# gunrock/graphblast

Hardware: NVIDIA H100
Metric: MTEPS (higher is better)
Workload: dtype f32

## Files before the change

### graphblast_b200/csrc/graphblas/backend/cuda/bfs_fused.hpp

```cpp
#ifndef GRAPHBLAS_BACKEND_CUDA_BFS_FUSED_HPP_
#define GRAPHBLAS_BACKEND_CUDA_BFS_FUSED_HPP_

#include "graphblas/backend/cuda/kernels/bfs_fused.cuh"

namespace graphblas {
namespace backend {

inline bool bfsFusedApplies(Descriptor* desc) {
  static const int enabled = getEnv("GB200_BFS_FUSED", 1);
  if (!enabled) return false;
  Desc_value mask_mode, outp, inp0, inp1;
  if (desc->get(GrB_MASK, &mask_mode) != GrB_SUCCESS) return false;
  desc->get(GrB_OUTP, &outp); desc->get(GrB_INP0, &inp0); desc->get(GrB_INP1, &inp1);
  return desc->struconly() && desc->opreuse() && desc->earlyexit() && desc->fusedmask() &&
         mask_mode == GrB_DEFAULT && outp == GrB_DEFAULT && inp0 == GrB_DEFAULT &&
         inp1 == GrB_DEFAULT && !desc->debug() && desc->timing_ != 1;
}

inline void bfsFusedStats(Descriptor* desc, Index n, unsigned long long out[6]) {
  for (int i = 0; i < 6; ++i) out[i] = 0ull;
  const size_t nwords = (static_cast<size_t>(n) + 31)/32;
  const size_t words_bytes = ((nwords*sizeof(unsigned int) + 255)/256)*256;
  if (desc->scratchSize(GB_SCRATCH_BFS) < 4*words_bytes + 256) return;
  unsigned char* base = reinterpret_cast<unsigned char*>(desc->scratch(GB_SCRATCH_BFS, 0));
  CUDA_CALL(cudaMemcpyAsync(out, base + 4*words_bytes + 6*sizeof(unsigned long long),
      6*sizeof(unsigned long long), cudaMemcpyDeviceToHost, gbStream()));
  runtime().sync();
}

template <typename a>
Info bfsFused(Vector<float>* v, const Matrix<a>* A, Index s, Descriptor* desc, int* depth) {
  SparseMatrix<a>* S = const_cast<SparseMatrix<a>*>(&A->sparse_);
  const Index n = S->nrows_;
  if (n != S->ncols_) return GrB_DIMENSION_MISMATCH;
  if (S->d_csrRowPtr_ == NULL || S->d_cscColPtr_ == NULL) return GrB_UNINITIALIZED_OBJECT;
  cudaStream_t stream = gbStream();
  CHECK(v->setStorage(GrB_DENSE));
  CHECK(v->dense_.allocateGpu());

  const int fw = 1;
  const Index* probe = pullMaxDegreeNeighbours(S, fw, S->d_cscColPtr_, S->d_cscRowInd_, n);

  const size_t nwords = (static_cast<size_t>(n) + 31)/32;
  const size_t words_bytes = ((nwords*sizeof(unsigned int) + 255)/256)*256;
  const size_t nchunks = (nwords + 31)/32;
  const size_t counters_bytes = GB_BFS_NCOUNTERS*sizeof(unsigned long long);
  const size_t heavy_bytes = GB_BFS_HEAVY_CAP*sizeof(Index);
  const size_t walk_bytes = nchunks*GB_BFS_CHUNK*sizeof(Index);
  const size_t lists_bytes = ((nchunks*(sizeof(int) + sizeof(Index)) + 255)/256)*256;
  const size_t level8_bytes = ((static_cast<size_t>(n) + 255)/256)*256;
  unsigned char* base = reinterpret_cast<unsigned char*>(desc->scratch(GB_SCRATCH_BFS,
      4*words_bytes + counters_bytes + heavy_bytes + walk_bytes + lists_bytes +
      level8_bytes));
  BfsFusedArgs args;
  args.push_ptr = S->d_csrRowPtr_;  args.push_ind = S->d_csrColInd_;
  args.pull_ptr = S->d_cscColPtr_;  args.pull_ind = S->d_cscRowInd_;
  args.pull_probe = probe;
  const bool same_structure = S->symmetric_ || S->d_cscColPtr_ == S->d_csrRowPtr_;
  args.pull_empty = pullEmptyRowBits(probe, n);
  args.push_empty = same_structure ? NULL : pullEmptyRowBits(
      pullFirstNeighbours(S, 0, S->d_csrRowPtr_, S->d_csrColInd_, n), n);
  args.n = n;
  args.source = s;
  args.max_levels = desc->max_niter_;
  args.switchpoint = desc->switchpoint();
  Desc_value mode;
  CHECK(desc->get(GrB_MXVMODE, &mode));
  args.mode = (mode == GrB_PUSHONLY) ? 1 : (mode == GrB_PULLONLY ? 2 : 0);
  args.levels = v->dense_.d_val_;
  args.visited[0] = reinterpret_cast<unsigned int*>(base);
  args.visited[1] = reinterpret_cast<unsigned int*>(base + words_bytes);
  args.frontier   = reinterpret_cast<unsigned int*>(base + 2*words_bytes);
  args.next       = reinterpret_cast<unsigned int*>(base + 3*words_bytes);
  args.counters   = reinterpret_cast<unsigned long long*>(base + 4*words_bytes);
  args.heavy      = reinterpret_cast<Index*>(base + 4*words_bytes + counters_bytes);
  args.walk       = reinterpret_cast<Index*>(base + 4*words_bytes + counters_bytes +
                                             heavy_bytes);
  args.walk_count = reinterpret_cast<int*>(base + 4*words_bytes + counters_bytes +
                                           heavy_bytes + walk_bytes);
  args.walk_chunks = reinterpret_cast<Index*>(args.walk_count + nchunks);
  args.level8     = base + 4*words_bytes + counters_bytes + heavy_bytes + walk_bytes +
                    lists_bytes;

  static const int trace = getEnv("GB200_BFS_TRACE", 0);
  args.trace = trace;
  args.prof_bytes = NULL;
  if (profiler().enabled) {
    profiler().ensureCells();
    args.prof_bytes = profiler().d_cells + GB_PROF_PULL_BOOL;
  }

  const bool push_only = (args.mode == 1);
  void (*kernel)(BfsFusedArgs) =
      push_only ? bfsFusedKernel<GB_BFS_PUSH_NT, GB_BFS_PUSH_MINB, false>
                : bfsFusedKernel<GB_BFS_NT, GB_BFS_MINB, true>;
  const int nt = push_only ? GB_BFS_PUSH_NT : GB_BFS_NT;
  static int resident_of[2] = {0, 0};
  int& resident = resident_of[push_only ? 1 : 0];
  if (resident == 0) {
    int per_sm = 0;
    CUDA_CALL(cudaOccupancyMaxActiveBlocksPerMultiprocessor(&per_sm, kernel, nt, 0));
    resident = per_sm*runtime().sm_count;
    if (resident < 1) return GrB_PANIC;
  }
  void* params[] = { &args };
  profiler().begin(GB_PROF_PULL_BOOL, stream);
  CUDA_CALL(cudaLaunchCooperativeKernel(reinterpret_cast<void*>(kernel),
      dim3(resident), dim3(nt), params, 0, stream));
  GB_KERNEL_CHECK();
  profiler().end(GB_PROF_PULL_BOOL, stream, 0.0);
  v->dense_.touched();
  if (trace) {
    unsigned long long cells[GB_BFS_NCOUNTERS];
    CUDA_CALL(cudaMemcpyAsync(cells, args.counters, sizeof(cells), cudaMemcpyDeviceToHost,
        stream));
    runtime().sync();
    const int levels = static_cast<int>(cells[6] < 15 ? cells[6] : 15);
    fprintf(stderr, "bfs trace: set-up %.1fus",
            1e-3*static_cast<double>((cells[12] >> 1) - cells[28]));
    for (int l = 1; l <= levels; ++l) {
      const unsigned long long start = cells[12 + l - 1] >> 1, end = cells[12 + l] >> 1;
      if (cells[12 + l] & 1ull)
        fprintf(stderr, " L%d pull %.1fus (scan %.1f walk %.1f, %llu walked, %llu listed)",
                l, 1e-3*static_cast<double>(end - start),
                1e-3*static_cast<double>(cells[44 + l] - start),
                1e-3*static_cast<double>(end - cells[44 + l]), cells[60 + l],
                cells[76 + l]);
      else
        fprintf(stderr, " L%d push %.1fus", l, 1e-3*static_cast<double>(end - start));
    }
    fprintf(stderr, " end-pass %.1fus\n", 1e-3*static_cast<double>(cells[29] - cells[30]));
  }
  if (depth != NULL) {
    const unsigned long long levels = runtime().fetch(args.counters + 6);
    *depth = static_cast<int>(levels);
    desc->lastmxv_ = GrB_PULLONLY;
  }
  return GrB_SUCCESS;
}

}
}

#endif
```

### graphblast_b200/csrc/graphblas/backend/cuda/kernels/bfs_fused.cuh

```cuda
#ifndef GRAPHBLAS_BACKEND_CUDA_KERNELS_BFS_FUSED_CUH_
#define GRAPHBLAS_BACKEND_CUDA_KERNELS_BFS_FUSED_CUH_

#include <cooperative_groups.h>

#include "graphblas/backend/cuda/kernels/common.cuh"

namespace graphblas {
namespace backend {

#ifndef GB_BFS_NT
#define GB_BFS_NT     512
#endif
#ifndef GB_BFS_MINB
#define GB_BFS_MINB   2
#endif
#ifndef GB_BFS_PUSH_NT
#define GB_BFS_PUSH_NT   768
#endif
#ifndef GB_BFS_PUSH_MINB
#define GB_BFS_PUSH_MINB 2
#endif
#ifndef GB_BFS_BATCH
#define GB_BFS_BATCH  4
#endif
#ifndef GB_BFS_WALK_STEP
#define GB_BFS_WALK_STEP 4
#endif
#ifndef GB_BFS_WALK_WARP
#define GB_BFS_WALK_WARP 32
#endif
#ifndef GB_BFS_WALK_INLINE
#define GB_BFS_WALK_INLINE 64
#endif
#define GB_BFS_HEAVY  2048
#define GB_BFS_HEAVY_CAP 4096
#define GB_BFS_CHUNK  1024

struct BfsFusedArgs {
  const Index* push_ptr;   const Index* push_ind;
  const Index* pull_ptr;   const Index* pull_ind;
  const Index* pull_probe;
  const unsigned int* pull_empty;
  const unsigned int* push_empty;
  int   trace;
  unsigned long long* prof_bytes;
  Index n;
  Index source;
  int   max_levels;
  float switchpoint;
  int   mode;
  float*        levels;
  unsigned char* level8;
  unsigned int* visited[2];
  unsigned int* frontier;
  unsigned int* next;
  unsigned long long* counters;
  Index*        heavy;
  Index*        walk;
  int*          walk_count;
  Index*        walk_chunks;
};
#define GB_BFS_NCOUNTERS 128

__device__ __forceinline__ unsigned long long bfsClockNs() {
  unsigned long long t;
  asm volatile("mov.u64 %0, %globaltimer;" : "=l"(t));
  return t;
}

__device__ __forceinline__ bool bfsClaim(unsigned int* visited, Index vtx) {
  const unsigned int bit = 1u << (vtx & 31);
  unsigned int* word = visited + (vtx >> 5);
  if (*reinterpret_cast<volatile unsigned int*>(word) & bit) return false;
  return (atomicOr(word, bit) & bit) == 0;
}

__device__ __forceinline__ void bfsSetLevel(const BfsFusedArgs& a, Index row, int lv) {
  if (lv < 255) {
    a.level8[row] = static_cast<unsigned char>(lv);
  } else {
    a.level8[row] = 255;
    a.levels[row] = static_cast<float>(lv);
  }
}

__device__ __forceinline__ Index bfsClaimChunk(unsigned long long* cell, int lane) {
  unsigned long long c = 0ull;
  if (lane == 0) c = atomicAdd(cell, 1ull);
  return static_cast<Index>(__shfl_sync(GB_FULL_MASK, c, 0));
}

__device__ __forceinline__ unsigned int* bfsVis(const BfsFusedArgs& a, int vsel) {
  return vsel ? a.visited[1] : a.visited[0];
}
__device__ __forceinline__ unsigned int* bfsVisOther(const BfsFusedArgs& a, int vsel) {
  return vsel ? a.visited[0] : a.visited[1];
}
__device__ __forceinline__ unsigned int* bfsF(const BfsFusedArgs& a, int fsel) {
  return fsel ? a.next : a.frontier;
}
__device__ __forceinline__ unsigned int* bfsN(const BfsFusedArgs& a, int fsel) {
  return fsel ? a.frontier : a.next;
}

__device__ __forceinline__ unsigned int bfsIsolated(const BfsFusedArgs& a, Index w) {
  return a.pull_empty[w] & (a.push_empty != NULL ? a.push_empty[w] : 0xffffffffu);
}

__device__ __forceinline__ bool bfsWalkRows(const BfsFusedArgs& a, int vsel, Index row,
                                            bool active, int lane, int& inspected) {
  Index k = 0, end = 0;
  if (active) {
    k = __ldg(a.pull_ptr + row);
    end = __ldg(a.pull_ptr + row + 1);
  }
  const Index stop = (end - k > GB_BFS_WALK_WARP + GB_BFS_WALK_STEP)
                     ? k + GB_BFS_WALK_STEP : end;
  bool found = false;
  while (k < stop && !found) {
    Index col[GB_BFS_WALK_STEP];
    unsigned int wv[GB_BFS_WALK_STEP];
#pragma unroll
    for (int u = 0; u < GB_BFS_WALK_STEP; ++u)
      col[u] = (k + u < stop) ? __ldg(a.pull_ind + k + u) : static_cast<Index>(-1);
#pragma unroll
    for (int u = 0; u < GB_BFS_WALK_STEP; ++u)
      wv[u] = (col[u] >= 0) ? bfsVis(a, vsel)[col[u] >> 5] : 0u;
#pragma unroll
    for (int u = 0; u < GB_BFS_WALK_STEP; ++u) {
      if (found || col[u] < 0) continue;
      ++inspected;
      found = (wv[u] >> (col[u] & 31)) & 1u;
    }
    k += GB_BFS_WALK_STEP;
  }
  unsigned int longs = __ballot_sync(GB_FULL_MASK, !found && k < end);
  while (longs != 0u) {
    const int src = __ffs(longs) - 1;
    longs &= longs - 1u;
    const Index lend = __shfl_sync(GB_FULL_MASK, end, src);
    bool hit = false;
    for (Index lk = __shfl_sync(GB_FULL_MASK, k, src); lk < lend && !hit; lk += 32) {
      bool v = false;
      if (lk + lane < lend) {
        const Index col = __ldg(a.pull_ind + lk + lane);
        v = (bfsVis(a, vsel)[col >> 5] >> (col & 31)) & 1u;
      }
      const unsigned int b = __ballot_sync(GB_FULL_MASK, v);
      hit = (b != 0u);
      if (lane == 0)
        inspected += hit ? __ffs(b) : (lend - lk < 32 ? lend - lk : 32);
    }
    if (lane == src) found = hit;
  }
  return found;
}

template <int NT, int MINB, bool PULL>
__global__ void __launch_bounds__(NT, MINB)
bfsFusedKernel(BfsFusedArgs a) {
  namespace cg = cooperative_groups;
  cg::grid_group grid = cg::this_grid();
  __shared__ int s_red[NT/32];
  __shared__ unsigned int s_found[PULL ? NT/32 : 1][PULL ? 32 : 1];

  const Index n = a.n;
  const Index nwords = (n + 31) >> 5;
  const int lane = threadIdx.x & 31;
  const Index gtid = blockIdx.x*NT + threadIdx.x;
  const Index gthreads = gridDim.x*NT;
  const Index gwarp = gtid >> 5;
  const Index gwarps = gthreads >> 5;
  const Index nchunks = (nwords + 31) >> 5;

  if (gtid == 0) a.counters[28] = bfsClockNs();
  if (gtid == 0) a.level8[a.source] = 1;
  for (Index w = gtid; w < nwords; w += gthreads) {
    const unsigned int seed = (w == (a.source >> 5)) ? (1u << (a.source & 31)) : 0u;
    a.visited[0][w] = seed | bfsIsolated(a, w);
    a.visited[1][w] = 0u; a.frontier[w] = seed; a.next[w] = 0u;
  }
  if (gtid < 12) a.counters[gtid] = 0ull;
  if (gtid >= 35 && gtid < 41) a.counters[gtid] = 0ull;
  if (gtid >= 60 && gtid < 76) a.counters[gtid] = 0ull;
  grid.sync();
  if (gtid == 0) a.counters[12] = bfsClockNs() << 1;

  int vsel = 0;
  int fsel = 0;
  unsigned int fcount = 1u;
  bool dense = PULL && (a.mode == 2);
  float prev_ratio = 0.f;
  int inspected = 0;
  int pushed_vertices = 0;
  unsigned int pushed_edges = 0u;
  int pull_levels = 0;
  int level = 1;

  for (; level <= a.max_levels && fcount > 0u; ++level) {
    if (PULL && a.mode == 0) {
      const float ratio = static_cast<float>(fcount)/static_cast<float>(n);
      if (!dense) {
        if (ratio > a.switchpoint && ratio > prev_ratio) dense = true; else prev_ratio = ratio;
      } else {
        if (ratio <= a.switchpoint && ratio < prev_ratio) dense = false; else prev_ratio = ratio;
      }
    }
    unsigned long long* const count_cell = a.counters + (level % 3);
    unsigned long long* const heavy_cell = a.counters + 3 + (level % 3);
    if (gtid == 0) {
      a.counters[(level + 1) % 3] = 0ull;
      a.counters[3 + (level + 1) % 3] = 0ull;
      a.counters[35 + (level + 1) % 3] = 0ull;
      a.counters[38 + (level + 1) % 3] = 0ull;
    }
    int found_here = 0;

    if (!dense) {
      for (Index w0 = gwarp*32; w0 < nwords; w0 += gwarps*32) {
        const Index mine = w0 + lane;
        unsigned int my_bits = (mine < nwords) ? bfsF(a, fsel)[mine] : 0u;
        if (my_bits != 0u) bfsF(a, fsel)[mine] = 0u;
        unsigned int pending = __ballot_sync(GB_FULL_MASK, my_bits != 0u);
        while (pending != 0u) {
          const int src_lane = __ffs(pending) - 1;
          pending &= pending - 1u;
          unsigned int bits = __shfl_sync(GB_FULL_MASK, my_bits, src_lane);
          const Index w = w0 + src_lane;
          while (bits != 0u) {
            const int b = __ffs(bits) - 1;
            bits &= bits - 1u;
            const Index u = w*32 + b;
            const Index beg = __ldg(a.push_ptr + u);
            const Index deg = __ldg(a.push_ptr + u + 1) - beg;
            if (lane == 0) { ++pushed_vertices; pushed_edges += deg; }
            if (deg > GB_BFS_HEAVY) {
              unsigned long long slot = 0ull;
              if (lane == 0) slot = atomicAdd(heavy_cell, 1ull);
              slot = __shfl_sync(GB_FULL_MASK, slot, 0);
              if (slot < GB_BFS_HEAVY_CAP) {
                if (lane == 0) a.heavy[slot] = u;
                continue;
              }
            }
            for (Index k = lane; k < deg; k += 32) {
              const Index nbr = __ldg(a.push_ind + beg + k);
              if (bfsClaim(bfsVis(a, vsel), nbr)) {
                bfsSetLevel(a, nbr, level + 1);
                atomicOr(bfsN(a, fsel) + (nbr >> 5), 1u << (nbr & 31));
                ++found_here;
              }
            }
          }
        }
      }
      grid.sync();
      const unsigned long long listed =
          *reinterpret_cast<volatile unsigned long long*>(heavy_cell);
      const int nheavy = (listed > GB_BFS_HEAVY_CAP) ? GB_BFS_HEAVY_CAP
                                                     : static_cast<int>(listed);
      if (nheavy > 0) {
        for (int h = 0; h < nheavy; ++h) {
          const Index u = a.heavy[h];
          const Index beg = __ldg(a.push_ptr + u);
          const Index deg = __ldg(a.push_ptr + u + 1) - beg;
          for (Index k = gtid; k < deg; k += gthreads) {
            const Index nbr = __ldg(a.push_ind + beg + k);
            if (bfsClaim(bfsVis(a, vsel), nbr)) {
              bfsSetLevel(a, nbr, level + 1);
              atomicOr(bfsN(a, fsel) + (nbr >> 5), 1u << (nbr & 31));
              ++found_here;
            }
          }
        }
      }
    } else if (PULL) {
      ++pull_levels;
      unsigned long long* const walk_cell = a.counters + 35 + (level % 3);
      unsigned long long* const list_cell = a.counters + 38 + (level % 3);
      Index c = gwarp;
      unsigned int next_vis = (c < nchunks && c*32 + lane < nwords)
                              ? bfsVis(a, vsel)[c*32 + lane] : 0xffffffffu;
      while (c < nchunks) {
        const Index word = c*32 + lane;
        const unsigned int my_vis = next_vis;
        const Index c_next = c + gwarps;
        next_vis = (c_next < nchunks && c_next*32 + lane < nwords)
                   ? bfsVis(a, vsel)[c_next*32 + lane] : 0xffffffffu;
        Index* const walk = a.walk + c*GB_BFS_CHUNK;
        int nwalk = 0;
        unsigned int my_out = 0u;
        unsigned int open = __ballot_sync(GB_FULL_MASK, my_vis != 0xffffffffu);
        unsigned int my_open = ~my_vis;
        if (word == nwords - 1 && (n & 31) != 0) my_open &= (1u << (n & 31)) - 1u;
        const int nopen = __popc(my_open);
        int first = nopen;
#pragma unroll
        for (int off = 1; off < 32; off <<= 1) {
          const int t = __shfl_up_sync(GB_FULL_MASK, first, off);
          if (lane >= off) first += t;
        }
        const int total = __shfl_sync(GB_FULL_MASK, first, 31);
        first -= nopen;
        const int word_batches = (__popc(open) + GB_BFS_BATCH - 1)/GB_BFS_BATCH;
        const int row_batches = (total + 32*GB_BFS_BATCH - 1)/(32*GB_BFS_BATCH);
        if (2*row_batches < word_batches) {
          open = 0u;
          unsigned int* const found_bits = s_found[threadIdx.x >> 5];
          found_bits[lane] = 0u;
          __syncwarp();
          for (int r0 = 0; r0 < total; r0 += 32*GB_BFS_BATCH) {
            int local[GB_BFS_BATCH];
            Index f[GB_BFS_BATCH];
#pragma unroll
            for (int j = 0; j < GB_BFS_BATCH; ++j) {
              const int r = r0 + 32*j + lane;
              int wl = 0, base = 0;
#pragma unroll
              for (int step = 16; step > 0; step >>= 1) {
                const int fs = __shfl_sync(GB_FULL_MASK, first, wl + step);
                if (fs <= r) { wl += step; base = fs; }
              }
              unsigned int m = __shfl_sync(GB_FULL_MASK, my_open, wl);
              int k = r - base, b = 0;
#pragma unroll
              for (int width = 16; width > 0; width >>= 1) {
                const int lo = __popc(m & ((1u << width) - 1u));
                if (k >= lo) { k -= lo; b += width; m >>= width; }
              }
              local[j] = wl*32 + b;
              f[j] = (r < total) ? __ldg(a.pull_probe + c*GB_BFS_CHUNK + local[j])
                                 : static_cast<Index>(-1);
            }
            unsigned int pword[GB_BFS_BATCH];
#pragma unroll
            for (int j = 0; j < GB_BFS_BATCH; ++j)
              pword[j] = (f[j] != static_cast<Index>(-1))
                         ? bfsVis(a, vsel)[(f[j] & 0x7fffffff) >> 5] : 0u;
#pragma unroll
            for (int j = 0; j < GB_BFS_BATCH; ++j) {
              if (r0 + 32*j >= total) break;
              const bool found = (pword[j] >> (f[j] & 31)) & 1u;
              inspected += (f[j] != static_cast<Index>(-1)) ? 1 : 0;
              const bool walk_row = f[j] >= 0 && !found;
              const Index row = c*GB_BFS_CHUNK + local[j];
              const unsigned int walkers = __ballot_sync(GB_FULL_MASK, walk_row);
              if (walk_row) walk[nwalk + __popc(walkers & ((1u << lane) - 1u))] = row;
              nwalk += __popc(walkers);
              if (found) {
                atomicOr(found_bits + (local[j] >> 5), 1u << (local[j] & 31));
                bfsSetLevel(a, row, level + 1);
                ++found_here;
              }
            }
          }
          __syncwarp();
          my_out = found_bits[lane];
        }
        while (open != 0u) {
          const unsigned int batch = open;
          Index f[GB_BFS_BATCH];
#pragma unroll
          for (int j = 0; j < GB_BFS_BATCH; ++j) {
            const int wl = __ffs(open) - 1;
            open &= open - 1u;
            f[j] = static_cast<Index>(-1);
            if (wl >= 0) {
              const unsigned int m = __shfl_sync(GB_FULL_MASK, my_vis, wl);
              const Index row = c*GB_BFS_CHUNK + wl*32 + lane;
              if (row < n && !((m >> lane) & 1u)) f[j] = __ldg(a.pull_probe + row);
            }
          }
          unsigned int pword[GB_BFS_BATCH];
#pragma unroll
          for (int j = 0; j < GB_BFS_BATCH; ++j)
            pword[j] = (f[j] != static_cast<Index>(-1))
                       ? bfsVis(a, vsel)[(f[j] & 0x7fffffff) >> 5] : 0u;
          unsigned int hit = 0u, more = 0u;
#pragma unroll
          for (int j = 0; j < GB_BFS_BATCH; ++j) {
            const bool found = (pword[j] >> (f[j] & 31)) & 1u;
            inspected += (f[j] != static_cast<Index>(-1)) ? 1 : 0;
            hit |= static_cast<unsigned int>(found) << j;
            more |= static_cast<unsigned int>(f[j] >= 0 && !found) << j;
          }
          unsigned int rest = batch;
#pragma unroll
          for (int j = 0; j < GB_BFS_BATCH && rest != 0u; ++j) {
            const int wl = __ffs(rest) - 1;
            rest &= rest - 1u;
            const Index row = c*GB_BFS_CHUNK + wl*32 + lane;
            const bool found = (hit >> j) & 1u, walk_row = (more >> j) & 1u;
            const unsigned int walkers = __ballot_sync(GB_FULL_MASK, walk_row);
            if (walk_row) walk[nwalk + __popc(walkers & ((1u << lane) - 1u))] = row;
            nwalk += __popc(walkers);
            const unsigned int out = __ballot_sync(GB_FULL_MASK, found);
            if (found) { bfsSetLevel(a, row, level + 1); ++found_here; }
            if (lane == wl) my_out = out;
          }
        }
        if (nwalk > 0 && nwalk <= GB_BFS_WALK_INLINE) {
          unsigned int* const found_bits = s_found[threadIdx.x >> 5];
          found_bits[lane] = my_out;
          __syncwarp();
          for (int i0 = 0; i0 < nwalk; i0 += 32) {
            const bool active = i0 + lane < nwalk;
            const Index row = active ? walk[i0 + lane] : 0;
            if (bfsWalkRows(a, vsel, row, active, lane, inspected)) {
              const int local = row & (GB_BFS_CHUNK - 1);
              atomicOr(found_bits + (local >> 5), 1u << (local & 31));
              bfsSetLevel(a, row, level + 1);
              ++found_here;
            }
          }
          __syncwarp();
          my_out = found_bits[lane];
        }
        if (word < nwords) {
          bfsN(a, fsel)[word] = my_out;
          bfsVisOther(a, vsel)[word] = my_vis | my_out;
          bfsF(a, fsel)[word] = 0u;
        }
        if (lane == 0 && nwalk > 0) {
          if (nwalk > GB_BFS_WALK_INLINE) {
            a.walk_count[c] = nwalk;
            a.walk_chunks[atomicAdd(list_cell, 1ull)] = c;
          }
          if (a.trace && level < 16)
            atomicAdd(a.counters + 60 + level, static_cast<unsigned long long>(nwalk));
        }
        c = c_next;
      }
      grid.sync();
      const Index nlisted = static_cast<Index>(
          *reinterpret_cast<volatile unsigned long long*>(list_cell));
      if (gtid == 0 && level < 16) {
        a.counters[44 + level] = bfsClockNs();
        if (a.trace) a.counters[76 + level] = static_cast<unsigned long long>(nlisted);
      }
      for (Index i = gwarp; i < nlisted; ) {
        const Index i_next = gwarps + bfsClaimChunk(walk_cell, lane);
        const Index c = a.walk_chunks[i];
        const int nwalk = a.walk_count[c];
        for (int i0 = 0; i0 < nwalk; i0 += 32) {
          const bool active = i0 + lane < nwalk;
          const Index row = active ? a.walk[c*GB_BFS_CHUNK + i0 + lane] : 0;
          if (bfsWalkRows(a, vsel, row, active, lane, inspected)) {
            const unsigned int bit = 1u << (row & 31);
            atomicOr(bfsN(a, fsel) + (row >> 5), bit);
            atomicOr(bfsVisOther(a, vsel) + (row >> 5), bit);
            bfsSetLevel(a, row, level + 1);
            ++found_here;
          }
        }
        i = i_next;
      }
    }
    const int block_found = blockSum<NT>(found_here, s_red);
    if (threadIdx.x == 0 && block_found) {
      atomicAdd(count_cell, static_cast<unsigned long long>(block_found));
      if (!dense)
        atomicAdd(a.counters + 11, static_cast<unsigned long long>(block_found));
    }
    grid.sync();
    if (gtid == 0 && level < 16)
      a.counters[12 + level] = (bfsClockNs() << 1) | (dense ? 1ull : 0ull);
    fcount = static_cast<unsigned int>(
        *reinterpret_cast<volatile unsigned long long*>(count_cell));
    if (dense) vsel ^= 1;
    fsel ^= 1;
  }
  if (gtid == 0) a.counters[30] = bfsClockNs();
  const unsigned int* const cut_rows = (fcount > 0u) ? bfsF(a, fsel) : NULL;
  const bool lines = (reinterpret_cast<uintptr_t>(a.levels) & 15u) == 0u;
  const Index nblocks = (nwords + 15) >> 4;
  for (Index blk = gwarp; blk < nblocks; blk += gwarps) {
    const Index r0 = blk*512;
    const Index w = blk*16 + (lane & 15);
    unsigned int reached = 0u;
    if (lane < 16 && w < nwords) {
      reached = bfsVis(a, vsel)[w] & ~bfsIsolated(a, w);
      if (cut_rows != NULL) reached &= ~cut_rows[w];
      if (w == (a.source >> 5)) reached |= 1u << (a.source & 31);
    }
#pragma unroll
    for (int j = 0; j < 4; ++j) {
      const unsigned int bits =
          (__shfl_sync(GB_FULL_MASK, reached, 4*j + (lane >> 3)) >> (4*(lane & 7))) & 0xfu;
      const Index row = r0 + 128*j + 4*lane;
      if (row >= n) continue;
      if (lines && row + 4 <= n) {
        const unsigned int b = *reinterpret_cast<const unsigned int*>(a.level8 + row);
        float f[4];
        bool escape = false;
#pragma unroll
        for (int k = 0; k < 4; ++k) {
          const unsigned int byte = (b >> (8*k)) & 0xffu;
          const bool r = (bits >> k) & 1u;
          escape |= r && byte == 255u;
          f[k] = r ? static_cast<float>(byte) : 0.f;
        }
        if (!escape) {
          *reinterpret_cast<float4*>(a.levels + row) = make_float4(f[0], f[1], f[2], f[3]);
          continue;
        }
      }
      for (int k = 0; k < 4 && row + k < n; ++k) {
        if (!((bits >> k) & 1u)) {
          a.levels[row + k] = 0.f;
        } else {
          const unsigned int byte = a.level8[row + k];
          if (byte != 255u) a.levels[row + k] = static_cast<float>(byte);
        }
      }
    }
  }
  if (a.trace) {
    grid.sync();
    if (gtid == 0) a.counters[29] = bfsClockNs();
  }
  const int block_insp = blockSum<NT>(inspected, s_red);
  const int block_pv = blockSum<NT>(pushed_vertices, s_red);
  if (threadIdx.x == 0) {
    if (block_insp) atomicAdd(a.counters + 7, static_cast<unsigned long long>(block_insp));
    if (block_pv)   atomicAdd(a.counters + 9, static_cast<unsigned long long>(block_pv));
  }
  if (pushed_edges) atomicAdd(a.counters + 10, static_cast<unsigned long long>(pushed_edges));
  if (gtid == 0) {
    a.counters[6] = static_cast<unsigned long long>(level - 1);
    a.counters[8] = static_cast<unsigned long long>(pull_levels);
  }
  if (a.prof_bytes != NULL) {
    if (pushed_edges) atomicAdd(a.prof_bytes, 8ull*pushed_edges);
    if (threadIdx.x == 0) {
      unsigned long long bytes = 4ull*static_cast<unsigned long long>(block_insp) +
                                 12ull*static_cast<unsigned long long>(block_pv);
      if (blockIdx.x == 0)
        bytes += static_cast<unsigned long long>(pull_levels)*
                     (12ull*static_cast<unsigned long long>(n) + 4ull) +
                 8ull*(*reinterpret_cast<volatile unsigned long long*>(a.counters + 11));
      if (bytes) atomicAdd(a.prof_bytes, bytes);
    }
  }
}

}
}

#endif
```

### graphblast_b200/csrc/graphblas/backend/cuda/pull_summary.hpp

```cpp
#ifndef GRAPHBLAS_BACKEND_CUDA_PULL_SUMMARY_HPP_
#define GRAPHBLAS_BACKEND_CUDA_PULL_SUMMARY_HPP_

namespace graphblas {
namespace backend {

template <typename T>
const Index* pullFirstNeighbours(SparseMatrix<T>* S, int side, const Index* ptr,
                                 const Index* ind, Index nrows) {
  if (S->d_pull_first_[side] == NULL || S->pull_first_key_[side] != ptr ||
      S->pull_first_nvals_[side] != S->nvals_) {
    if (S->d_pull_first_[side] != NULL) gbFree(S->d_pull_first_[side]);
    const size_t nwords = (static_cast<size_t>(nrows) + 31)/32;
    S->d_pull_first_[side] = reinterpret_cast<Index*>(
        gbMalloc((static_cast<size_t>(nrows) + 1 + nwords)*sizeof(Index)));
    cudaStream_t s = gbStream();
    pullFirstNeighbourKernel<<<gridFor(nrows, 256, 8), 256, 0, s>>>(
        S->d_pull_first_[side], ptr, ind, nrows);
    GB_KERNEL_CHECK();
    pullEmptyRowBitsKernel<<<gridFor(nrows, 256, 8), 256, 0, s>>>(
        reinterpret_cast<unsigned int*>(S->d_pull_first_[side] + nrows + 1),
        S->d_pull_first_[side], nrows);
    GB_KERNEL_CHECK();
    S->pull_first_key_[side] = ptr;
    S->pull_first_nvals_[side] = S->nvals_;
  }
  return S->d_pull_first_[side];
}

template <typename T>
const Index* pullMaxDegreeNeighbours(SparseMatrix<T>* S, int side, const Index* ptr,
                                     const Index* ind, Index nrows) {
  if (S->d_pull_maxdeg_[side] == NULL || S->pull_maxdeg_key_[side] != ptr ||
      S->pull_maxdeg_nvals_[side] != S->nvals_) {
    if (S->d_pull_maxdeg_[side] != NULL) gbFree(S->d_pull_maxdeg_[side]);
    const size_t nwords = (static_cast<size_t>(nrows) + 31)/32;
    S->d_pull_maxdeg_[side] = reinterpret_cast<Index*>(
        gbMalloc((static_cast<size_t>(nrows) + 1 + nwords)*sizeof(Index)));
    cudaStream_t s = gbStream();
    pullMaxDegreeNeighbourKernel<<<gridFor(static_cast<size_t>(nrows)*32, 256, 8), 256, 0,
                                   s>>>(S->d_pull_maxdeg_[side], ptr, ind, nrows);
    GB_KERNEL_CHECK();
    pullEmptyRowBitsKernel<<<gridFor(nrows, 256, 8), 256, 0, s>>>(
        reinterpret_cast<unsigned int*>(S->d_pull_maxdeg_[side] + nrows + 1),
        S->d_pull_maxdeg_[side], nrows);
    GB_KERNEL_CHECK();
    S->pull_maxdeg_key_[side] = ptr;
    S->pull_maxdeg_nvals_[side] = S->nvals_;
  }
  return S->d_pull_maxdeg_[side];
}

inline const unsigned int* pullEmptyRowBits(const Index* first, Index nrows) {
  return reinterpret_cast<const unsigned int*>(first + nrows + 1);
}

}
}

#endif
```

Measured before the change: 2.330 million.

## Probe pull rows in quad groups with vectorized int4 loads and direct level writes

Reworks the bottom-up probe loop so each lane handles four consecutive rows of an open word, loading their probe neighbours with one int4 load and handling four words per warp round instead of one row per lane per word. Hit masks are assembled with xor shuffles, walk-list appends are skipped when no lane needs them, and levels are written directly as bytes into level8. The batching heuristic changes to count quad rounds with a tunable row-cost factor. It adds an alignment guard and pads the probe allocation so the vector loads stay in bounds. In exchange it uses more shuffles per round and relies on my_open and alignment assumptions.

```diff
diff --git a/graphblast_b200/csrc/graphblas/backend/cuda/bfs_fused.hpp b/graphblast_b200/csrc/graphblas/backend/cuda/bfs_fused.hpp
--- a/graphblast_b200/csrc/graphblas/backend/cuda/bfs_fused.hpp
+++ b/graphblast_b200/csrc/graphblas/backend/cuda/bfs_fused.hpp
@@ -40,6 +40,7 @@
 
   const int fw = 1;
   const Index* probe = pullMaxDegreeNeighbours(S, fw, S->d_cscColPtr_, S->d_cscRowInd_, n);
+  if ((reinterpret_cast<uintptr_t>(probe) & 15u) != 0u) return GrB_PANIC;
 
   const size_t nwords = (static_cast<size_t>(n) + 31)/32;
   const size_t words_bytes = ((nwords*sizeof(unsigned int) + 255)/256)*256;
diff --git a/graphblast_b200/csrc/graphblas/backend/cuda/kernels/bfs_fused.cuh b/graphblast_b200/csrc/graphblas/backend/cuda/kernels/bfs_fused.cuh
--- a/graphblast_b200/csrc/graphblas/backend/cuda/kernels/bfs_fused.cuh
+++ b/graphblast_b200/csrc/graphblas/backend/cuda/kernels/bfs_fused.cuh
@@ -31,6 +31,9 @@
 #endif
 #ifndef GB_BFS_WALK_INLINE
 #define GB_BFS_WALK_INLINE 64
+#endif
+#ifndef GB_BFS_ROW_COST
+#define GB_BFS_ROW_COST 2
 #endif
 #define GB_BFS_HEAVY  2048
 #define GB_BFS_HEAVY_CAP 4096
@@ -302,9 +305,9 @@
         }
         const int total = __shfl_sync(GB_FULL_MASK, first, 31);
         first -= nopen;
-        const int word_batches = (__popc(open) + GB_BFS_BATCH - 1)/GB_BFS_BATCH;
+        const int quad_rounds = (__popc(open) + 3)/4;
         const int row_batches = (total + 32*GB_BFS_BATCH - 1)/(32*GB_BFS_BATCH);
-        if (2*row_batches < word_batches) {
+        if (GB_BFS_ROW_COST*row_batches < quad_rounds) {
           open = 0u;
           unsigned int* const found_bits = s_found[threadIdx.x >> 5];
           found_bits[lane] = 0u;
@@ -357,46 +360,62 @@
           __syncwarp();
           my_out = found_bits[lane];
         }
+        const int sub = 4*(lane & 7);
+        const bool q_odd = (lane >> 3) & 1, q_high = (lane >> 4) & 1;
+        const unsigned int below = (1u << lane) - 1u;
         while (open != 0u) {
-          const unsigned int batch = open;
-          Index f[GB_BFS_BATCH];
-#pragma unroll
-          for (int j = 0; j < GB_BFS_BATCH; ++j) {
-            const int wl = __ffs(open) - 1;
-            open &= open - 1u;
-            f[j] = static_cast<Index>(-1);
-            if (wl >= 0) {
-              const unsigned int m = __shfl_sync(GB_FULL_MASK, my_vis, wl);
-              const Index row = c*GB_BFS_CHUNK + wl*32 + lane;
-              if (row < n && !((m >> lane) & 1u)) f[j] = __ldg(a.pull_probe + row);
-            }
-          }
-          unsigned int pword[GB_BFS_BATCH];
-#pragma unroll
-          for (int j = 0; j < GB_BFS_BATCH; ++j)
-            pword[j] = (f[j] != static_cast<Index>(-1))
-                       ? bfsVis(a, vsel)[(f[j] & 0x7fffffff) >> 5] : 0u;
-          unsigned int hit = 0u, more = 0u;
-#pragma unroll
-          for (int j = 0; j < GB_BFS_BATCH; ++j) {
-            const bool found = (pword[j] >> (f[j] & 31)) & 1u;
-            inspected += (f[j] != static_cast<Index>(-1)) ? 1 : 0;
-            hit |= static_cast<unsigned int>(found) << j;
-            more |= static_cast<unsigned int>(f[j] >= 0 && !found) << j;
-          }
-          unsigned int rest = batch;
-#pragma unroll
-          for (int j = 0; j < GB_BFS_BATCH && rest != 0u; ++j) {
-            const int wl = __ffs(rest) - 1;
-            rest &= rest - 1u;
-            const Index row = c*GB_BFS_CHUNK + wl*32 + lane;
-            const bool found = (hit >> j) & 1u, walk_row = (more >> j) & 1u;
-            const unsigned int walkers = __ballot_sync(GB_FULL_MASK, walk_row);
-            if (walk_row) walk[nwalk + __popc(walkers & ((1u << lane) - 1u))] = row;
-            nwalk += __popc(walkers);
-            const unsigned int out = __ballot_sync(GB_FULL_MASK, found);
-            if (found) { bfsSetLevel(a, row, level + 1); ++found_here; }
-            if (lane == wl) my_out = out;
+          const unsigned int o1 = open & (open - 1u), o2 = o1 & (o1 - 1u),
+                             o3 = o2 & (o2 - 1u);
+          const unsigned int round = open ^ (o3 & (o3 - 1u));
+          const unsigned int oq = q_high ? (q_odd ? o3 : o2) : (q_odd ? o1 : open);
+          open = o3 & (o3 - 1u);
+          const int wl = __ffs(oq) - 1;
+          const unsigned int m = __shfl_sync(GB_FULL_MASK, my_open, wl & 31);
+          const unsigned int mine = (oq != 0u) ? (m >> sub) & 0xfu : 0u;
+          const Index row0 = c*GB_BFS_CHUNK + wl*32 + sub;
+          int4 f4 = make_int4(-1, -1, -1, -1);
+          if (mine != 0u) f4 = __ldg(reinterpret_cast<const int4*>(a.pull_probe + row0));
+          Index f[4] = {f4.x, f4.y, f4.z, f4.w};
+          const unsigned int* const vis = bfsVis(a, vsel);
+          unsigned int pword[4];
+#pragma unroll
+          for (int k = 0; k < 4; ++k) {
+            if (!((mine >> k) & 1u)) f[k] = static_cast<Index>(-1);
+            pword[k] = (f[k] != static_cast<Index>(-1)) ? vis[(f[k] & 0x7fffffff) >> 5] : 0u;
+          }
+          unsigned int probed = 0u, hit = 0u, more = 0u;
+#pragma unroll
+          for (int k = 0; k < 4; ++k) {
+            const bool found = (pword[k] >> (f[k] & 31)) & 1u;
+            probed |= static_cast<unsigned int>(f[k] != static_cast<Index>(-1)) << k;
+            hit |= static_cast<unsigned int>(found) << k;
+            more |= static_cast<unsigned int>(f[k] >= 0 && !found) << k;
+          }
+          inspected += __popc(probed);
+          found_here += __popc(hit);
+          unsigned int out = hit << sub;
+          out |= __shfl_xor_sync(GB_FULL_MASK, out, 1);
+          out |= __shfl_xor_sync(GB_FULL_MASK, out, 2);
+          out |= __shfl_xor_sync(GB_FULL_MASK, out, 4);
+          out = __shfl_sync(GB_FULL_MASK, out, (8*__popc(round & below)) & 31);
+          if ((round >> lane) & 1u) my_out = out;
+          if (__any_sync(GB_FULL_MASK, more != 0u)) {
+#pragma unroll
+            for (int k = 0; k < 4; ++k) {
+              const unsigned int bk = __ballot_sync(GB_FULL_MASK, (more >> k) & 1u);
+              if ((more >> k) & 1u) walk[nwalk + __popc(bk & below)] = row0 + k;
+              nwalk += __popc(bk);
+            }
+          }
+          if (level + 1 < 255) {
+            unsigned char* const bytes = a.level8 + row0;
+#pragma unroll
+            for (int k = 0; k < 4; ++k)
+              if ((hit >> k) & 1u) bytes[k] = static_cast<unsigned char>(level + 1);
+          } else {
+#pragma unroll
+            for (int k = 0; k < 4; ++k)
+              if ((hit >> k) & 1u) bfsSetLevel(a, row0 + k, level + 1);
           }
         }
         if (nwalk > 0 && nwalk <= GB_BFS_WALK_INLINE) {
diff --git a/graphblast_b200/csrc/graphblas/backend/cuda/pull_summary.hpp b/graphblast_b200/csrc/graphblas/backend/cuda/pull_summary.hpp
--- a/graphblast_b200/csrc/graphblas/backend/cuda/pull_summary.hpp
+++ b/graphblast_b200/csrc/graphblas/backend/cuda/pull_summary.hpp
@@ -35,7 +35,7 @@
     if (S->d_pull_maxdeg_[side] != NULL) gbFree(S->d_pull_maxdeg_[side]);
     const size_t nwords = (static_cast<size_t>(nrows) + 31)/32;
     S->d_pull_maxdeg_[side] = reinterpret_cast<Index*>(
-        gbMalloc((static_cast<size_t>(nrows) + 1 + nwords)*sizeof(Index)));
+        gbMalloc((static_cast<size_t>(nrows) + 1 + nwords + 3)*sizeof(Index)));
     cudaStream_t s = gbStream();
     pullMaxDegreeNeighbourKernel<<<gridFor(static_cast<size_t>(nrows)*32, 256, 8), 256, 0,
                                    s>>>(S->d_pull_maxdeg_[side], ptr, ind, nrows);
```

Result: faster. 2.359 million, median of 6 (+1.3%).
